# Tomeu7/AO-MARL

Measured on AMD Instinct MI355X. Metric: env steps/sec (AO frames/sec), higher is better.
Workload: dtype f32

## Files before the change

### ao_marl_amd/csrc/aomarl_capi.hip

```cpp
#include "aomarl_kernels.hip"

#include <math.h>
#include <stdlib.h>
#include <stdarg.h>
#include <stdio.h>
#include <string.h>

#include <algorithm>
#include <climits>
#include <string>
#include <vector>

static thread_local char g_err[512] = "";

int fail(const char *fmt, ...) {
  va_list ap;
  va_start(ap, fmt);
  vsnprintf(g_err, sizeof(g_err), fmt, ap);
  va_end(ap);
  return 1;
}


struct aomarl_ctx {
  DevSys sys;
  std::vector<void *> owned;
  int nlayers = 0, ndm = 0;
  int dim[AOMARL_MAX_LAYERS], ns[AOMARL_MAX_LAYERS], abclass[AOMARL_MAX_LAYERS];
  float deltax[AOMARL_MAX_LAYERS], deltay[AOMARL_MAX_LAYERS];
  int nclass = 0;
  int maxdim = 0, maxK = 0;
  float gain = 0.f, delay = 0.f;
  bool spot_fast = false;
  bool force_generic_dm = false, force_valu_target = false;
  bool force_generic_spot = false, force_generic_target = false, force_unfused_frame = false;
  int dft_mode = -1;
  bool reset_untransposed = false;
  int small_chain = 1;
  hipEvent_t ride_ev = nullptr;
  bool rode = false;
  int residual_shortcut = 0;
  bool skip_do_control = false;
  int small_move = 1;
  bool small_ok = false;
  int reset_streams = 2;
  bool reset_prefetch_whole = true;
  hipEvent_t ev_reset = nullptr, ev_reset2[3] = {nullptr, nullptr, nullptr};
  bool no_extrude_sg = false;
  bool defer_dm_shape = false;
  int fused_debug = 0;
  bool prefetch_atmos = false, premoved = false;
  bool frame_wait_pending = false;
  bool screens_dirty_main = true;
  float cmat_scale = 1.f, v2m_scale = 1.f, m2v_scale = 1.f, s2m_scale = 1.f, ab_scale[AOMARL_MAX_LAYERS] = {1.f, 1.f, 1.f, 1.f, 1.f, 1.f, 1.f, 1.f};
  bool subpixel_flow = false;
  float frac_x[AOMARL_MAX_LAYERS] = {0, 0, 0, 0, 0, 0, 0, 0}, frac_y[AOMARL_MAX_LAYERS] = {0, 0, 0, 0, 0, 0, 0, 0};
  bool graph_step = false, capturing = false, side_joined = false, fork_recorded = false;
  hipEvent_t ev_fork = nullptr;
  struct StepGraph { std::vector<long long> key; hipGraphExec_t exec; hipGraph_t graph; unsigned long long arith[AR_N]; int fw_variant[6]; };
  std::vector<StepGraph> graphs;
  unsigned long long graph_hits = 0, graph_captures = 0;
  unsigned long long cfg_epoch = 0;
  const int32_t *sel_checked = nullptr;
  int sel_checked_n = 0, sel_checked_nm = 0;
  int fw_variant[6] = {0, 0, 0, 0, 0, 0};
  char fw_name[96] = {0};
  bool time_fw = false;
  std::vector<hipEvent_t> fw_ev;
  size_t fw_ev_used = 0;
  std::vector<hipEvent_t> fw_ev_retired;
  hipStream_t atm_stream = nullptr, psf_stream = nullptr;
  hipEvent_t ev_frame = nullptr, ev_moved = nullptr, ev_psf = nullptr;
  hipEvent_t ev_frame_cur = nullptr;
  bool frame_marked = false;
  struct FramePipe {
    bool have_twin = false, active = false;
    const float *owner_screens = nullptr;
    aomarl_state twin;
    int par = 0;
    hipStream_t fstream = nullptr;
    hipEvent_t ev_cmd = nullptr, ev_commit = nullptr, ev_done[2] = {nullptr, nullptr}, ev_psf[2] = {nullptr, nullptr};
    hipEvent_t ev_done_cur[2] = {nullptr, nullptr};
    bool psf_out[2] = {false, false};
// ... 396 lines not shown
      std::vector<int32_t> tinfo(tsub.size(), 0);
      for (int r = 0; r < nt; r++)
        for (int t = 0; t < nt; t++) {
          const int32_t sb = tsub[(size_t)r * nt + t];
          bool full = true;
          for (int yy = 0; yy < 16; yy++) full = full && tmask[(size_t)(16 * r + yy) * nt + t] == 0xFFFF;
          int32_t v = 0;
          if (sb != -2) v |= 0x10000;
          if (full) v |= 0x20000;
          if (sb >= 0) { v |= 0x40000 | sb; v |= 0x10000; }
          tinfo[(size_t)r * nt + t] = v;
        }
      UP(int32_t, tinfo.data(), tinfo.size(), s.tile_info);
      {
        if (nt > 127) { aomarl_destroy(c); return fail("pupil too wide for the frame kernel's tile list"); }
        std::vector<int32_t> linfo((size_t)nt * (nt + 8), 0), lcount(nt, 0);
        for (int r = 0; r < nt; r++) {
          int k = 0;
          for (int t = 0; t < nt; t++)
            if (tinfo[(size_t)r * nt + t] & 0x10000) linfo[(size_t)r * (nt + 8) + k++] = tinfo[(size_t)r * nt + t] | (t << 24);
          lcount[r] = k;
          for (int kk = k; kk < nt + 8; kk++) linfo[(size_t)r * (nt + 8) + kk] = k ? linfo[(size_t)r * (nt + 8) + k - 1] : 0;
        }
        UP(int32_t, linfo.data(), linfo.size(), s.lit_info);
        UP(int32_t, lcount.data(), lcount.size(), s.lit_count);
        const int npm = (nt + 1) / 2 + 2;
        std::vector<int32_t> pinfo((size_t)nt * npm * 2, 0), pcount(nt, 0);
        for (int r = 0; r < nt; r++) {
          int k = 0;
          int32_t *row = &pinfo[(size_t)r * npm * 2];
          for (int g = 0; 2 * g < nt; g++) {
            const int ta = 2 * g, tb = 2 * g + 1 < nt ? 2 * g + 1 : 2 * g;
            const int32_t va = tinfo[(size_t)r * nt + ta], vb = 2 * g + 1 < nt ? tinfo[(size_t)r * nt + tb] : 0;
            if (!((va | vb) & 0x10000)) continue;
            row[2 * k] = ((va & 0x10000) ? va : 0) | (ta << 24);
            row[2 * k + 1] = ((vb & 0x10000) ? vb : 0) | (tb << 24);
            k++;
          }
          pcount[r] = k;
          for (int kk = k; kk < npm; kk++) {
            row[2 * kk] = k ? row[2 * (k - 1)] : 0;
            row[2 * kk + 1] = k ? row[2 * (k - 1) + 1] : 0;
          }
        }
        UP(int32_t, pinfo.data(), pinfo.size(), s.pair_info);
        UP(int32_t, pcount.data(), pcount.size(), s.pair_count);
      }
      {
        std::vector<int32_t> order(nt), work(nt, 0);
        for (int r = 0; r < nt; r++) {
          order[r] = r;
          for (int t = 0; t < nt; t++) {
            const int32_t v = tinfo[(size_t)r * nt + t];
            work[r] += (v & 0x10000) ? ((v & 0x40000) ? 4 : 1) : 0;
          }
        }
        std::stable_sort(order.begin(), order.end(), [&](int a, int b) { return work[a] > work[b]; });
        UP(int32_t, order.data(), order.size(), s.stripe_order);
      }
      {
        std::vector<_Float16> tw((size_t)nt * 64 * 8);
        std::vector<float> twf((size_t)nt * 64 * 4);
        for (int t = 0; t < nt; t++)
          for (int lane = 0; lane < 64; lane++)
            for (int j = 0; j < 4; j++) {
              const int x = 16 * t + 4 * (lane >> 4) + j, cc = lane & 15;
              const int k = cc < 8 ? cc + 1 : cc - 7;
              const double th = 2.0 * M_PI * (double)(((long long)k * x) % d->npsf) / (double)d->npsf;
              const float v = (float)(cc < 8 ? cos(th) : sin(th));
              const _Float16 hi = (_Float16)v;
              const _Float16 lo = (_Float16)(v - (float)hi);
              _Float16 *o = &tw[((size_t)t * 64 + lane) * 8];
              o[j] = hi; o[4 + j] = lo;
              twf[((size_t)t * 64 + lane) * 4 + j] = v;
            }
        const _Float16 *dev = nullptr;
        UP(_Float16, tw.data(), tw.size(), dev);
        s.psf_tw_h = dev;
        const float *devf = nullptr;
        UP(float, twf.data(), twf.size(), devf);
        s.psf_tw_f = devf;
      }
      {
        std::vector<float> z(64 * 8, 0.f);
        float *qt;
        UP(float, z.data(), z.size(), qt);
        hipLaunchKernelGGL(k_fill_qf_tab, dim3(1), dim3(128), 0, 0, qt);
        if (hipGetLastError() != hipSuccess || hipDeviceSynchronize() != hipSuccess) { aomarl_destroy(c); return fail("create: quadratic-form constants"); }
        s.qf_tab = qt;
      }
      UP(uint16_t, tmask.data(), tmask.size(), s.tile_mask);
      {
        const DevDm &T = s.dms[1];
        std::vector<float> tp((size_t)pd * pd * 2);
        for (int y = 0; y < pd; y++)
          for (int g = 0; g < pd / 4; g++)
            for (int j = 0; j < 4; j++) {
              const size_t o = (size_t)(y + T.toy) * T.dim + T.tox + 4 * g + j;
              float *dst = &tp[((size_t)y * (pd / 4) + g) * 8];
              dst[j] = c->h_tt[2 * o]; dst[4 + j] = c->h_tt[2 * o + 1];
            }
        UP(float, tp.data(), tp.size(), s.tt_pk);
      }
      s.fused_ok = 1; s.ntiles = nt;
      const DevDm &Z = s.dms[0];
      s.otf_ok = 0;
      if (Z.sep && Z.pitch > 0 && 16 % Z.pitch == 0) {
        auto first = [&](int p0, int pmin) {
          const int num = p0 - pmin - (Z.ss - 1);
          return num >= 0 ? (num + Z.pitch - 1) / Z.pitch : -((-num) / Z.pitch);
        };
        s.otf_gx0 = first(Z.tox, Z.i1min); s.otf_gy0 = first(Z.toy, Z.j1min);
        s.otf_xoff = Z.tox - (Z.i1min + Z.pitch * s.otf_gx0);
        s.otf_yoff = Z.toy - (Z.j1min + Z.pitch * s.otf_gy0);
        const int cnt = std::max((s.otf_xoff + 15) / Z.pitch + 1, (s.otf_yoff + 15) / Z.pitch + 1);
        s.otf_nb = (cnt + 3) / 4; s.otf_tpn = 16 / Z.pitch;
        s.otf_latw = (nt - 1) * s.otf_tpn + 4 * s.otf_nb;
        s.otf_ok = (s.otf_nb >= 1 && s.otf_nb <= 2 && s.otf_xoff >= 0 && s.otf_yoff >= 0) ? 1 : 0;
      }
    }
  }
#undef UP
  *out = c;
  return 0;
}

int aomarl_destroy(aomarl_ctx *c) {
  if (c)
    for (auto &sg : c->graphs) { (void)hipGraphExecDestroy(sg.exec); (void)hipGraphDestroy(sg.graph); }
  if (c) c->graphs.clear();
  if (!c) return 0;
  for (void *p : c->owned) (void)hipFree(p);
  for (int k = 0; k < 2; k++) {
    if (c->pipe.snap[k]) (void)hipFree(c->pipe.snap[k]);
    if (c->pipe.ev_done[k]) (void)hipEventDestroy(c->pipe.ev_done[k]);
    if (c->pipe.ev_psf[k]) (void)hipEventDestroy(c->pipe.ev_psf[k]);
  }
  if (c->ev_reset) (void)hipEventDestroy(c->ev_reset);
  for (int k = 0; k < 3; k++) if (c->ev_reset2[k]) (void)hipEventDestroy(c->ev_reset2[k]);
  if (c->pipe.ev_cmd) (void)hipEventDestroy(c->pipe.ev_cmd);
  if (c->pipe.ev_commit) (void)hipEventDestroy(c->pipe.ev_commit);
  if (c->pipe.fstream) { (void)hipStreamSynchronize(c->pipe.fstream); (void)hipStreamDestroy(c->pipe.fstream); }
  if (c->atm_stream) (void)hipStreamSynchronize(c->atm_stream);
  if (c->psf_stream) (void)hipStreamSynchronize(c->psf_stream);
  if (c->ev_frame) (void)hipEventDestroy(c->ev_frame);
  if (c->ev_moved) (void)hipEventDestroy(c->ev_moved);
  if (c->ev_psf) (void)hipEventDestroy(c->ev_psf);
  if (c->env_gain) (void)hipFree(c->env_gain);
  if (c->seed_stage) (void)hipFree(c->seed_stage);
  rp_free(c);
  if (c->timg) (void)hipFree(c->timg);
  for (hipEvent_t e : c->fw_ev) (void)hipEventDestroy(e);
  for (hipEvent_t e : c->fw_ev_retired) (void)hipEventDestroy(e);
  delete c;
  return 0;
}

static int replace_dev(aomarl_ctx *c, float **slot, const std::vector<float> &h) {
  if (*slot) {
    for (size_t i = 0; i < c->owned.size(); i++)
      if (c->owned[i] == *slot) { c->owned.erase(c->owned.begin() + i); break; }
    (void)hipFree(*slot);
    *slot = nullptr;
  }
  return upload<float>(c, h.data(), h.size(), slot);
}

int aomarl_set_cmat(aomarl_ctx *c, const float *cmat) {
  if (c) c->cfg_epoch++;
  if (!c || !cmat) return fail("aomarl_set_cmat: null argument");
  const int na = c->sys.nactu, nsl = c->sys.nslope;
// ... 176 lines not shown
```

### ao_marl_amd/csrc/aomarl_kernels.hip

```cpp
#include "aomarl_host.h"
#include "aomarl_gemm_p.h"
#include <type_traits>

#define WAVE 64

typedef unsigned u32x4 __attribute__((ext_vector_type(4)));

__device__ __forceinline__ hx2 cvt_h2(float a, float b) {
  return __builtin_bit_cast(hx2, __builtin_amdgcn_cvt_pkrtz(a, b));
}
__device__ __forceinline__ float sub_lo(hx2 h, float a) {
  float r;
  asm("v_fma_mix_f32 %0, %1, -1.0, %2 op_sel_hi:[1,0,0]" : "=v"(r) : "v"(h), "v"(a));
  return r;
}
__device__ __forceinline__ float sub_hi(hx2 h, float a) {
  float r;
  asm("v_fma_mix_f32 %0, %1, -1.0, %2 op_sel:[1,0,0] op_sel_hi:[1,0,0]" : "=v"(r) : "v"(h), "v"(a));
  return r;
}

struct __attribute__((packed, aligned(4))) f4u { float v[4]; };
__device__ __forceinline__ void add4(float acc[4], const float *p) {
  const f4u t = *reinterpret_cast<const f4u *>(p);
// ... 1368 lines not shown
  f32x2 d;
  asm volatile("v_pk_fma_f32 %0, %1, %2, %3" : "=v"(d) : "v"(a), "s"(bs), "v"(c));
  return d;
}
__device__ __forceinline__ f32x2 pk_fma_nc_s(f32x2 a, f32x2 bs, f32x2 c) {
  f32x2 d;
  asm volatile("v_pk_fma_f32 %0, %1, %2, %3 neg_lo:[0,0,1] neg_hi:[0,0,1]" : "=v"(d) : "v"(a), "s"(bs), "v"(c));
  return d;
}
__device__ __forceinline__ f32x2 pk_mul_s(f32x2 a, f32x2 bs) {
  f32x2 d;
  asm volatile("v_pk_mul_f32 %0, %1, %2" : "=v"(d) : "v"(a), "s"(bs));
  return d;
}

__device__ __forceinline__ void spot_cog_f32_pk(const DevSys &sys, const DevState &st, int e, int i, int lane,
                                                const float (&Cc)[4], const float (&Ss)[4], const float (&br)[4],
                                                const float (&bi)[4], int do_cog, const f32x4 z4) {
  const int q = lane >> 4, c = lane & 15;
  f32x4 PCr = z4, PCi = z4, PSr = z4, PSi = z4;
#pragma unroll
  for (int s = 0; s < 4; s++) {
    PCr = mfma16(br[s], Cc[s], PCr);
    PCi = mfma16(bi[s], Cc[s], PCi);
    PSr = mfma16(br[s], Ss[s], PSr);
    PSi = mfma16(bi[s], Ss[s], PSi);
  }
  PK_GUARD_MFMA();
  const f32x2 tr0l = pk_add(pk_lo(PCr), pk_lo(PSi)), ti0l = pk_sub(pk_lo(PCi), pk_lo(PSr));
  const f32x2 tr0h = pk_add(pk_hi(PCr), pk_hi(PSi)), ti0h = pk_sub(pk_hi(PCi), pk_hi(PSr));
  const f32x2 tr1l = pk_sub(pk_lo(PCr), pk_lo(PSi)), ti1l = pk_add(pk_lo(PCi), pk_lo(PSr));
  const f32x2 tr1h = pk_sub(pk_hi(PCr), pk_hi(PSi)), ti1h = pk_add(pk_hi(PCi), pk_hi(PSr));
  PK_END_TO_MFMA();
  const f32x4 TrA[2] = {pk_join(tr0l, tr0h), pk_join(tr1l, tr1h)};
  const f32x4 TiA[2] = {pk_join(ti0l, ti0h), pk_join(ti1l, ti1h)};
  f32x2 Pa[2], Pb[2];
  f32x2 Da, Db;
#pragma unroll
  for (int m = 0; m < 2; m++) {
    const f32x4 Tr = TrA[m], Ti = TiA[m];
    f32x4 QCr = z4, QCi = z4, QSr = z4, QSi = z4;
#pragma unroll
    for (int s = 0; s < 4; s++) {
      QCr = mfma16(Cc[s], Tr[s], QCr);
      QCi = mfma16(Cc[s], Ti[s], QCi);
      QSr = mfma16(Ss[s], Tr[s], QSr);
      QSi = mfma16(Ss[s], Ti[s], QSi);
    }
    PK_GUARD_MFMA();
    const f32x2 crl = pk_lo(QCr), crh = pk_hi(QCr), cil = pk_lo(QCi), cih = pk_hi(QCi);
    const f32x2 srl = pk_lo(QSr), srh = pk_hi(QSr), sil = pk_lo(QSi), sih = pk_hi(QSi);
    f32x2 pa = pk_mul(crl, crl), pb = pk_mul(crh, crh);
    if (m == 0) { Da = pk_mul(crl, sil); Db = pk_mul(crh, sih); }
    else { pk_acc_fma(Da, crl, sil); pk_acc_fma(Db, crh, sih); }
    pk_acc_fma(pa, sil, sil); pk_acc_fma(pb, sih, sih);
    pk_acc_fnma(Da, cil, srl); pk_acc_fnma(Db, cih, srh);
    pk_acc_fma(pa, cil, cil); pk_acc_fma(pb, cih, cih);
    pk_acc_fma(pa, srl, srl); pk_acc_fma(pb, srh, srh);
    Pa[m] = pa; Pb[m] = pb;
    __builtin_amdgcn_sched_barrier(0);
  }
  const f32x2 P0 = pk_add(Pa[0], Pb[0]), P1 = pk_add(Pa[1], Pb[1]);
  const float Xp = (float)(8 + (c >> 1)), Xm = (float)(7 - (c >> 1));
  const float p0 = P0.x + P0.y, p1 = P1.x + P1.y, da = Da.x + Da.y, db = Db.x + Db.y;
  float s0 = p0 + p1;
  float sx = fmaf(Xm, p1, Xp * p0);
  float sy = fmaf((float)(3 + 4 * q), db, fmaf((float)(1 + 4 * q), da, 7.5f * s0));
  s0 = wave_sum_last(s0);
  sx = wave_sum_last(sx);
  sy = wave_sum_last(sy);
  if (do_cog && lane == 63) {
    float *sl = st.slopes + (long long)e * sys.nslope;
    if (s0 > 0.f) {
      const float inv = __builtin_amdgcn_rcpf(s0);
      sl[i] = (sx * inv - sys.cog_offset) * sys.cog_scale;
      sl[sys.nvalid + i] = (sy * inv - sys.cog_offset) * sys.cog_scale;
    } else {
      sl[i] = 0.f;
      sl[sys.nvalid + i] = 0.f;
    }
  }
}

struct SpotQf { f32x2 Ml, Mh, Sl, Sh; };

__device__ __forceinline__ SpotQf spot_qf_consts(int lane, const float2 *sTw ) {
  const int q = lane >> 4, c = lane & 15;
  float m[4], sv[4];
#pragma unroll
  for (int s = 0; s < 4; s++) {
    const int d = c - (4 * q + s);
    float a = 0.f, b = 0.f;
    for (int j = 0; j < 16; j++) {
      const float2 w = sTw[((2 * j + 1) * d) & 127];
      a += w.x;
      b = fmaf(0.5f + (float)(j >> 1), w.y, b);
    }
    m[s] = (d != 0 && (d & 1) == 0) ? 0.f : 2.f * a;
    sv[s] = 2.f * b;
  }
  SpotQf k;
  k.Ml = f32x2{m[0], m[1]}; k.Mh = f32x2{m[2], m[3]};
  k.Sl = f32x2{sv[0], sv[1]}; k.Sh = f32x2{sv[2], sv[3]};
  return k;
}

__global__ __launch_bounds__(128) void k_fill_qf_tab(float *__restrict__ tab) {
  __shared__ float2 sTw[128];
  const int tid = threadIdx.x;
  float sn, cs;
  sincospif((float)tid * (1.0f / 64.0f), &sn, &cs);
  sTw[tid] = make_float2(cs, sn);
  __syncthreads();
  if (tid < 64) {
    const SpotQf k = spot_qf_consts(tid, sTw);
    float *o = tab + 8 * tid;
    o[0] = k.Ml.x; o[1] = k.Ml.y; o[2] = k.Mh.x; o[3] = k.Mh.y;
    o[4] = k.Sl.x; o[5] = k.Sl.y; o[6] = k.Sh.x; o[7] = k.Sh.y;
  }
}

typedef unsigned u32x2 __attribute__((ext_vector_type(2)));
#ifndef FW_QF6_PK
#define FW_QF6_PK 1
#endif
#ifndef FW_QF6_ACC2
#define FW_QF6_ACC2 0
#endif
__device__ __forceinline__ float swap32_add(float a, float b) {
  const u32x2 t = __builtin_amdgcn_permlane32_swap(__float_as_uint(a), __float_as_uint(b), false, false);
  return __uint_as_float(t[0]) + __uint_as_float(t[1]);
}
__device__ __forceinline__ float swap16_add(float a, float b) {
  const u32x2 t = __builtin_amdgcn_permlane16_swap(__float_as_uint(a), __float_as_uint(b), false, false);
  return __uint_as_float(t[0]) + __uint_as_float(t[1]);
}
__device__ __forceinline__ float spot_qf_moments(const SpotQf &K, const float (&er)[4], const float (&ei)[4], const f32x4 z4) {
  const float Mc[4] = {K.Ml.x, K.Ml.y, K.Mh.x, K.Mh.y}, Sc[4] = {K.Sl.x, K.Sl.y, K.Sh.x, K.Sh.y};
  f32x4 Wr = z4, Wi = z4, V = z4;
#pragma unroll
  for (int s = 0; s < 4; s++) {
    Wr = mfma16(Mc[s], er[s], Wr);
    Wi = mfma16(Mc[s], ei[s], Wi);
    V = mfma16(Sc[s], er[s], V);
  }
#if FW_QF6_PK
  const f32x2 er01 = {er[0], er[1]}, er23 = {er[2], er[3]}, ei01 = {ei[0], ei[1]}, ei23 = {ei[2], ei[3]};
  __builtin_amdgcn_sched_barrier(0);
  const f32x2 a01 = pk_add(er01, ei01), a23 = pk_add(er23, ei23);
  const f32x2 b01 = pk_sub(ei01, er01), b23 = pk_sub(ei23, er23);
  PK_END_TO_MFMA();
  const float A[4] = {a01.x, a01.y, a23.x, a23.y}, B[4] = {b01.x, b01.y, b23.x, b23.y};
#else
  float A[4], B[4];
#pragma unroll
  for (int s = 0; s < 4; s++) { A[s] = er[s] + ei[s]; B[s] = ei[s] - er[s]; }
#endif
#if FW_QF6_ACC2
  f32x4 Xa = z4, Xb = z4, G3 = z4;
#pragma unroll
  for (int s = 0; s < 4; s++) {
    Xa = mfma16(A[s], Wr[s], Xa);
    Xb = mfma16(B[s], Wi[s], Xb);
    G3 = mfma16(ei[s], V[s], G3);
  }
  PK_GUARD_MFMA();
  const f32x2 Xl = pk_add(pk_lo(Xa), pk_lo(Xb)), Xh = pk_add(pk_hi(Xa), pk_hi(Xb));
#else
  f32x4 X = z4, G3 = z4;
#pragma unroll
  for (int s = 0; s < 4; s++) {
    X = mfma16(A[s], Wr[s], X);
    G3 = mfma16(ei[s], V[s], G3);
    X = mfma16(B[s], Wi[s], X);
  }
  PK_GUARD_MFMA();
  const f32x2 Xl = pk_lo(X), Xh = pk_hi(X);
#endif
  f32x2 p0 = pk_mul(Xl, K.Ml);
  f32x2 px = pk_mul(pk_lo(G3), K.Ml);
  f32x2 py = pk_mul(Xl, K.Sl);
  pk_acc_fma(p0, Xh, K.Mh);
  pk_acc_fma(px, pk_hi(G3), K.Mh);
  pk_acc_fma(py, Xh, K.Sh);
  const float s0 = p0.x + p0.y, tx = px.x + px.y, ty = py.x + py.y;
  float z = swap16_add(swap32_add(s0, tx), swap32_add(ty, p0.y));
  z += dpp_f<0xB1>(z);
  z += dpp_f<0x4E>(z);
  z += dpp_f<0x141>(z);
  z += dpp_f<0x140>(z);
  return z;
}
__device__ __forceinline__ void qf_slopes(const DevSys &sys, float s0, float tx, float ty, float &sx, float &sy) {
  if (s0 > 0.f) {
    const float inv = __builtin_amdgcn_rcpf(s0);
    sx = (fmaf(tx, 2.f * inv, 7.5f) - sys.cog_offset) * sys.cog_scale;
    sy = (fmaf(-ty, inv, 7.5f) - sys.cog_offset) * sys.cog_scale;
  } else {
    sx = 0.f; sy = 0.f;
  }
}

template <bool NOISE, bool WRITE_CUBE>
__device__ __forceinline__ void spot_finish_v(const DevSys &sys, const DevState &st, int e, int i,
                                              int lane, const float (&v)[2][2][2], int do_cog,
                                              float flux_i) {
  const int q = lane >> 4, c = lane & 15;
  const bool owner = (c & 1) == 0;
  float tot = 0.f;
#pragma unroll
  for (int sy = 0; sy < 2; sy++)
#pragma unroll
    for (int sx = 0; sx < 2; sx++)
#pragma unroll
      for (int h = 0; h < 2; h++) tot += v[sy][sx][h];
  const int Xp = 8 + (c >> 1), Xm = 7 - (c >> 1);
  if (!NOISE && !WRITE_CUBE) {
    const float A0 = (v[0][0][0] + v[0][0][1]) + (v[1][0][0] + v[1][0][1]);
    const float A1 = (v[0][1][0] + v[0][1][1]) + (v[1][1][0] + v[1][1][1]);
    float sx_ = (float)Xp * A0;
    sx_ = fmaf((float)Xm, A1, sx_);
    float sy_ = (float)(8 + 2 * q) * (v[0][0][0] + v[0][1][0]);
    sy_ = fmaf((float)(9 + 2 * q), v[0][0][1] + v[0][1][1], sy_);
    sy_ = fmaf((float)(7 - 2 * q), v[1][0][0] + v[1][1][0], sy_);
    sy_ = fmaf((float)(6 - 2 * q), v[1][0][1] + v[1][1][1], sy_);
    tot = wave_sum_last(A0 + A1);
    sx_ = wave_sum_last(sx_);
    sy_ = wave_sum_last(sy_);
    if (do_cog && lane == 63) {
      float *sl = st.slopes + (long long)e * sys.nslope;
      if (tot > 0.f) {
        const float inv = __builtin_amdgcn_rcpf(tot);
        sl[i] = (sx_ * inv - sys.cog_offset) * sys.cog_scale;
        sl[sys.nvalid + i] = (sy_ * inv - sys.cog_offset) * sys.cog_scale;
      } else {
        sl[i] = 0.f;
        sl[sys.nvalid + i] = 0.f;
      }
    }
    (void)flux_i;
    return;
  }
  tot = wave_sum(owner ? tot : 0.f);
  const float g = tot > 0.f ? sys.nphot * flux_i / tot : 0.f;
  float s0 = 0.f, sx = 0.f, sy = 0.f;
  if (NOISE) {
    const int hh = c & 1;
    const uint32_t sd = st.seeds[e], fr = st.frame[e];
#pragma unroll
    for (int ty_ = 0; ty_ < 2; ty_++)
#pragma unroll
      for (int tx_ = 0; tx_ < 2; tx_++) {
        const int Y = ty_ ? 7 - (2 * q + hh) : 8 + 2 * q + hh, X = tx_ ? Xm : Xp;
        const uint32_t idx = (uint32_t)i * 256u + (uint32_t)(Y * 16 + X);
        const float val = sh_noise((hh ? v[ty_][tx_][1] : v[ty_][tx_][0]) * g, sys.noise, sd, fr, idx);
        if (WRITE_CUBE) st.bincube[((long long)e * sys.nvalid + i) * 256 + Y * 16 + X] = val;
        s0 += val;
        sx += val * (float)X;
        sy += val * (float)Y;
      }
  } else {
#pragma unroll
    for (int ty_ = 0; ty_ < 2; ty_++)
#pragma unroll
      for (int tx_ = 0; tx_ < 2; tx_++)
#pragma unroll
        for (int h = 0; h < 2; h++) {
          const int Y = ty_ ? 7 - (2 * q + h) : 8 + 2 * q + h, X = tx_ ? Xm : Xp;
// ... 417 lines not shown
#define FW_FULL 0x20000
#define FW_SUB 0x40000
__device__ __forceinline__ float sci_rev(float ph, float inv_lambda) { return ph * inv_lambda; }

typedef const int __attribute__((address_space(4))) *const_int_p;
typedef const float __attribute__((address_space(4))) *const_float_p;

template <int NL, bool OTF>
struct FrameRaw {
  float L[NL][4];
  float P[OTF ? 1 : 4], T[8];
  unsigned mrow;
  float F;
  f4u SH;
  float4 CS;
};

template <int NL, int NB, bool OTF, bool NOISE, bool WRITE_CUBE, bool HP>
#ifndef FW_WAVES
#define FW_WAVES 3
#endif
#ifndef FW_QF
#define FW_QF 1
#endif
#ifndef FW_DMA
#define FW_DMA 1
#endif
#ifndef FW_DEPTH
#define FW_DEPTH 2
#endif
#ifndef FW_DMA_F32
#define FW_DMA_F32 1
#endif
#ifndef FW_SLOTS1
#define FW_SLOTS1 0
#endif
#define FW_SLOT_BYTES(dma) ((dma) ? (FW_SLOTS1 ? 2 * 3 * 1024 : 16384) : 16384)
#define FWD_BLK 1152
#define FWD_IMG (2 * 1024 + 128)
#define FWD_WAVE(nl) ((nl) * FWD_IMG)
__global__ __launch_bounds__(256) __attribute__((amdgpu_waves_per_eu(FW_WAVES, FW_WAVES)))
void k_frame_wave(DevSys sys, DevState st, int env_begin,
                                                    int env_count, int do_cog,
                                                    float *__restrict__ TR,
                                                    float *__restrict__ TPART, int nblk) {
  extern __shared__ float smem[];
  const int pd = sys.pupdiam, ntl = sys.ntiles;
  const int tid = threadIdx.x, lane = tid & 63, q = lane >> 4, c = lane & 15;
  const int wv = __builtin_amdgcn_readfirstlane(tid >> 6);
  constexpr bool QF = FW_QF && OTF && !HP && !NOISE && !WRITE_CUBE;
  constexpr bool DMA = FW_DMA && OTF && (HP || FW_DMA_F32);
  float2 *sTw = reinterpret_cast<float2 *>(smem);
  float *lat_all = reinterpret_cast<float *>(sTw + (QF ? 0 : 128));
  float4 *shb = reinterpret_cast<float4 *>(lat_all + 4 * 4 * NB * (OTF ? sys.otf_latw : 0));
  char *dimg = reinterpret_cast<char *>(shb) + FW_SLOT_BYTES(DMA) + (DMA ? wv * FWD_WAVE(NL) : 0);
  float4 *qmom = reinterpret_cast<float4 *>(reinterpret_cast<char *>(shb) + FW_SLOT_BYTES(DMA) + (DMA ? 4 * FWD_WAVE(NL) : 0)) + wv * ntl;
  const int dbg = do_cog >> 8;
  do_cog &= 1;
  const int r = sys.stripe_order[blockIdx.y];
  const int el = 4 * blockIdx.x + wv;
  if constexpr (!QF) {
    if (tid < 128) {
      float sn, cs;
      sincospif((float)tid * (1.0f / 64.0f), &sn, &cs);
      sTw[tid] = make_float2(cs, sn);
    }
    __syncthreads();
  }
  const bool active = el < env_count;
  const int e = env_begin + (active ? el : env_count - 1);
  float Cc[4] = {0.f, 0.f, 0.f, 0.f}, Ss[4] = {0.f, 0.f, 0.f, 0.f};
  if constexpr (!QF) {
#pragma unroll
    for (int s = 0; s < 4; s++) {
      const float2 w = sTw[((4 * q + s) * (2 * c + 1)) & 127];
      Cc[s] = w.x; Ss[s] = w.y;
    }
  }
  SpotTwH twh;
  if (HP) twh = spot_tw_h(Cc, Ss);
  SpotQf qfk;
  if constexpr (QF) {
    const float4 ka = reinterpret_cast<const float4 *>(sys.qf_tab)[2 * lane], kb = reinterpret_cast<const float4 *>(sys.qf_tab)[2 * lane + 1];
    qfk.Ml = f32x2{ka.x, ka.y}; qfk.Mh = f32x2{ka.z, ka.w};
    qfk.Sl = f32x2{kb.x, kb.y}; qfk.Sh = f32x2{kb.z, kb.w};
  }
  unsigned shstep;
  const int y = 16 * r + c;
  const char *layb[NL];
  __amdgpu_buffer_rsrc_t lrs[NL];
  unsigned lpxs[NL], ldim[NL], lvo[NL];
#pragma unroll
  for (int l = 0; l < NL; l++) {
    const DevLayer &L = sys.layers[l];
    layb[l] = reinterpret_cast<const char *>(st.screens + (long long)e * sys.screen_stride + L.screen_off);
    lrs[l] = __builtin_amdgcn_make_buffer_rsrc(const_cast<char *>(layb[l]), 0,
                                               4 * L.dim * (L.dim + RING_PAD), 0x00020000);
    ldim[l] = (unsigned)L.dim;
    int px = L.tox + st.origin[(e * sys.nlayers + l) * 2]; px -= (px >= L.dim) ? L.dim : 0;
    int py = L.toy + st.origin[(e * sys.nlayers + l) * 2 + 1]; py -= (py >= L.dim) ? L.dim : 0;
    lpxs[l] = (unsigned)px;
    unsigned pr = (unsigned)y + (unsigned)py; pr = min(pr, pr - ldim[l]);
    lvo[l] = 4u * (pr * (ldim[l] + RING_PAD) + 4u * (unsigned)q);
  }
  const DevDm &D0 = sys.dms[0], &D1 = sys.dms[1];
  const float *pzt = st.dm_shape + (long long)e * sys.shape_stride + D0.shape_off;
  const float *ttslot = st.dm_shape + (long long)e * sys.shape_stride + D1.shape_off;
  const float c0 = ttslot[0], c1 = ttslot[1];
  const int half = pd / 2;
  const unsigned pvo = 4u * ((unsigned)(y + D0.toy) * (unsigned)D0.dim + (unsigned)D0.tox + 4u * (unsigned)q);
  const unsigned tvo = 32u * ((unsigned)y * (unsigned)(pd >> 2) + (unsigned)q);
  const unsigned mvo = 2u * (unsigned)y * (unsigned)ntl;
  const char *pztb = reinterpret_cast<const char *>(pzt);
  const char *ttb = reinterpret_cast<const char *>(sys.tt_pk);
  const char *mkb = reinterpret_cast<const char *>(sys.tile_mask);
  const bool sh_tt = wv < 2;
  const void *shbase = sh_tt ? static_cast<const void *>(ttb) : (HP ? sys.psf_tw_h : sys.psf_tw_f);
  const __amdgpu_buffer_rsrc_t shrs = __builtin_amdgcn_make_buffer_rsrc(
      const_cast<void *>(shbase), 0, sh_tt ? 8 * pd * pd : ntl * 1024, 0x00020000);
  const unsigned shvo = sh_tt ? tvo + 16u * (unsigned)wv : 16u * (unsigned)lane;
  shstep = sh_tt ? 7u : 10u;
  float pivot;
  {
    float v = OTF ? ttslot[2] : pzt[(half + D0.toy) * D0.dim + half + D0.tox];
    const float2 f = reinterpret_cast<const float2 *>(D1.influ)[(half + D1.toy) * D1.dim + half + D1.tox];
    v += c0 * f.x + c1 * f.y;
#pragma unroll
    for (int l = 0; l < NL; l++) {
      const DevLayer &L = sys.layers[l];
      int py = L.toy + st.origin[(e * sys.nlayers + l) * 2 + 1]; py -= (py >= L.dim) ? L.dim : 0;
      unsigned pyc = (unsigned)(half + py); pyc = min(pyc, pyc - ldim[l]);
      unsigned pxc = (unsigned)half + lpxs[l]; pxc = min(pxc, pxc - ldim[l]);
      v += reinterpret_cast<const float *>(layb[l])[pyc * (ldim[l] + RING_PAD) + pxc];
    }
    pivot = v;
  }
  float Pxr[NB], Pyr[NB];
  const int jm = (c >> 2) + 4 * (c & 3);
  const bool jm_ok = jm < 4 * NB;
  const int latw = sys.otf_latw, tpn = sys.otf_tpn;
  float *lat = lat_all + wv * (4 * NB * latw);
  if (OTF) {
#pragma unroll
    for (int s = 0; s < NB; s++) {
      const int ax = sys.otf_xoff + c - D0.pitch * (q + 4 * s);
      const int ay = sys.otf_yoff + c - D0.pitch * (q + 4 * s);
      Pxr[s] = (ax >= 0 && ax < D0.ss) ? D0.prof[ax] : 0.f;
      Pyr[s] = (ay >= 0 && ay < D0.ss) ? D0.prof[ay] : 0.f;
    }
    const float *volt = st.voltage + (long long)e * st.ld_actu + D0.com_off;
    for (int i = 0; i < 4 * NB; i++) {
      const int gy = sys.otf_gy0 + r * tpn + i;
      for (int jj = lane; jj < latw; jj += 64) {
        const int gx = sys.otf_gx0 + jj;
        float v = 0.f;
        if (gx >= 0 && gx < D0.gw && gy >= 0 && gy < D0.gh) {
          const int a = D0.grid[gy * D0.gw + gx];
          if (a >= 0) v = volt[a];
        }
        lat[i * latw + jj] = v;
      }
    }
    __builtin_amdgcn_wave_barrier();
  }
  const float *latq = lat + (jm_ok ? jm : 0);
  const float wfs_il = sys.wfs_inv_lambda, tar_il = sys.tar_inv_lambda;
  const f32x4 Z4 = opaque_zero4();
  f32x4 PA = {0.f, 0.f, 0.f, 0.f}, PB = {0.f, 0.f, 0.f, 0.f};
// ... 1146 lines not shown
```

Measured before the change: 549,900.

## Factor spot quadratic-form moments through a host-built orthogonal basis

Replaces the quadratic-form moment computation with a factorization: a symmetric basis H (from SVD and Jacobi eigen-decomposition on the host) projects the field, and the moments become sums of squares and cross terms of the projected vectors. The kernel goes from 20 MFMAs plus packed add/sub to 16 MFMAs and a few DPP multiply-accumulates, with constants built once on the host instead of by a setup kernel. It adds a fair amount of host numerical code and relies on the factorization reproducing the original moments to within float rounding.

Measured after the change: 570,500, median of 6. 1.04x the previous value.

```diff
diff --git a/ao_marl_amd/csrc/aomarl_capi.hip b/ao_marl_amd/csrc/aomarl_capi.hip
--- a/ao_marl_amd/csrc/aomarl_capi.hip
+++ b/ao_marl_amd/csrc/aomarl_capi.hip
@@ -1,4 +1,5 @@
 #include "aomarl_kernels.hip"
+#include "aomarl_qf4_host.h"
 
 #include <math.h>
 #include <stdlib.h>
@@ -561,11 +562,10 @@
         s.psf_tw_f = devf;
       }
       {
-        std::vector<float> z(64 * 8, 0.f);
-        float *qt;
-        UP(float, z.data(), z.size(), qt);
-        hipLaunchKernelGGL(k_fill_qf_tab, dim3(1), dim3(128), 0, 0, qt);
-        if (hipGetLastError() != hipSuccess || hipDeviceSynchronize() != hipSuccess) { aomarl_destroy(c); return fail("create: quadratic-form constants"); }
+        float qtab[64 * 8];
+        if (!aomarl_qf4::build_table(qtab)) { aomarl_destroy(c); return fail("create: quadratic-form constants"); }
+        const float *qt = nullptr;
+        UP(float, qtab, 64 * 8, qt);
         s.qf_tab = qt;
       }
       UP(uint16_t, tmask.data(), tmask.size(), s.tile_mask);
diff --git a/ao_marl_amd/csrc/aomarl_kernels.hip b/ao_marl_amd/csrc/aomarl_kernels.hip
--- a/ao_marl_amd/csrc/aomarl_kernels.hip
+++ b/ao_marl_amd/csrc/aomarl_kernels.hip
@@ -1474,51 +1474,9 @@
   }
 }
 
-struct SpotQf { f32x2 Ml, Mh, Sl, Sh; };
-
-__device__ __forceinline__ SpotQf spot_qf_consts(int lane, const float2 *sTw ) {
-  const int q = lane >> 4, c = lane & 15;
-  float m[4], sv[4];
-#pragma unroll
-  for (int s = 0; s < 4; s++) {
-    const int d = c - (4 * q + s);
-    float a = 0.f, b = 0.f;
-    for (int j = 0; j < 16; j++) {
-      const float2 w = sTw[((2 * j + 1) * d) & 127];
-      a += w.x;
-      b = fmaf(0.5f + (float)(j >> 1), w.y, b);
-    }
-    m[s] = (d != 0 && (d & 1) == 0) ? 0.f : 2.f * a;
-    sv[s] = 2.f * b;
-  }
-  SpotQf k;
-  k.Ml = f32x2{m[0], m[1]}; k.Mh = f32x2{m[2], m[3]};
-  k.Sl = f32x2{sv[0], sv[1]}; k.Sh = f32x2{sv[2], sv[3]};
-  return k;
-}
-
-__global__ __launch_bounds__(128) void k_fill_qf_tab(float *__restrict__ tab) {
-  __shared__ float2 sTw[128];
-  const int tid = threadIdx.x;
-  float sn, cs;
-  sincospif((float)tid * (1.0f / 64.0f), &sn, &cs);
-  sTw[tid] = make_float2(cs, sn);
-  __syncthreads();
-  if (tid < 64) {
-    const SpotQf k = spot_qf_consts(tid, sTw);
-    float *o = tab + 8 * tid;
-    o[0] = k.Ml.x; o[1] = k.Ml.y; o[2] = k.Mh.x; o[3] = k.Mh.y;
-    o[4] = k.Sl.x; o[5] = k.Sl.y; o[6] = k.Sh.x; o[7] = k.Sh.y;
-  }
-}
+struct SpotQf { f32x4 h; f32x2 ky; float kx; };
 
 typedef unsigned u32x2 __attribute__((ext_vector_type(2)));
-#ifndef FW_QF6_PK
-#define FW_QF6_PK 1
-#endif
-#ifndef FW_QF6_ACC2
-#define FW_QF6_ACC2 0
-#endif
 __device__ __forceinline__ float swap32_add(float a, float b) {
   const u32x2 t = __builtin_amdgcn_permlane32_swap(__float_as_uint(a), __float_as_uint(b), false, false);
   return __uint_as_float(t[0]) + __uint_as_float(t[1]);
@@ -1527,55 +1485,42 @@
   const u32x2 t = __builtin_amdgcn_permlane16_swap(__float_as_uint(a), __float_as_uint(b), false, false);
   return __uint_as_float(t[0]) + __uint_as_float(t[1]);
 }
+__device__ __forceinline__ float dpp4e_mul(float a, float b) {
+  float d;
+  asm volatile("v_mul_f32_dpp %0, %1, %2 quad_perm:[2,3,0,1] row_mask:0xf bank_mask:0xf bound_ctrl:1" : "=v"(d) : "v"(a), "v"(b));
+  return d;
+}
+__device__ __forceinline__ void dpp4e_fmac(float &acc, float a, float b) {
+  asm volatile("v_fmac_f32_dpp %0, %1, %2 quad_perm:[2,3,0,1] row_mask:0xf bank_mask:0xf bound_ctrl:1" : "+v"(acc) : "v"(a), "v"(b));
+}
 __device__ __forceinline__ float spot_qf_moments(const SpotQf &K, const float (&er)[4], const float (&ei)[4], const f32x4 z4) {
-  const float Mc[4] = {K.Ml.x, K.Ml.y, K.Mh.x, K.Mh.y}, Sc[4] = {K.Sl.x, K.Sl.y, K.Sh.x, K.Sh.y};
-  f32x4 Wr = z4, Wi = z4, V = z4;
+  f32x4 Dr = z4, Di = z4;
 #pragma unroll
   for (int s = 0; s < 4; s++) {
-    Wr = mfma16(Mc[s], er[s], Wr);
-    Wi = mfma16(Mc[s], ei[s], Wi);
-    V = mfma16(Sc[s], er[s], V);
-  }
-#if FW_QF6_PK
-  const f32x2 er01 = {er[0], er[1]}, er23 = {er[2], er[3]}, ei01 = {ei[0], ei[1]}, ei23 = {ei[2], ei[3]};
+    Dr = mfma16(er[s], K.h[s], Dr);
+    Di = mfma16(ei[s], K.h[s], Di);
+  }
+  f32x4 Pr = z4, Pi = z4;
+#pragma unroll
+  for (int r = 0; r < 4; r++) {
+    Pr = mfma16(K.h[r], Dr[r], Pr);
+    Pi = mfma16(K.h[r], Di[r], Pi);
+  }
+  PK_GUARD_MFMA();
+  const f32x2 rl = pk_lo(Pr), rh = pk_hi(Pr), il = pk_lo(Pi), ih = pk_hi(Pi);
+  f32x2 p0 = pk_mul(rl, rl);
+  f32x2 py = pk_mul(il, rh);
+  float px = dpp4e_mul(Pr[0], Pi[0]);
+  pk_acc_fma(p0, rh, rh);
+  pk_acc_fnma(py, ih, rl);
+  dpp4e_fmac(px, Pr[1], Pi[1]);
+  pk_acc_fma(p0, il, il);
+  py = pk_mul(py, K.ky);
+  dpp4e_fmac(px, Pr[2], Pi[2]);
+  pk_acc_fma(p0, ih, ih);
+  dpp4e_fmac(px, Pr[3], Pi[3]);
   __builtin_amdgcn_sched_barrier(0);
-  const f32x2 a01 = pk_add(er01, ei01), a23 = pk_add(er23, ei23);
-  const f32x2 b01 = pk_sub(ei01, er01), b23 = pk_sub(ei23, er23);
-  PK_END_TO_MFMA();
-  const float A[4] = {a01.x, a01.y, a23.x, a23.y}, B[4] = {b01.x, b01.y, b23.x, b23.y};
-#else
-  float A[4], B[4];
-#pragma unroll
-  for (int s = 0; s < 4; s++) { A[s] = er[s] + ei[s]; B[s] = ei[s] - er[s]; }
-#endif
-#if FW_QF6_ACC2
-  f32x4 Xa = z4, Xb = z4, G3 = z4;
-#pragma unroll
-  for (int s = 0; s < 4; s++) {
-    Xa = mfma16(A[s], Wr[s], Xa);
-    Xb = mfma16(B[s], Wi[s], Xb);
-    G3 = mfma16(ei[s], V[s], G3);
-  }
-  PK_GUARD_MFMA();
-  const f32x2 Xl = pk_add(pk_lo(Xa), pk_lo(Xb)), Xh = pk_add(pk_hi(Xa), pk_hi(Xb));
-#else
-  f32x4 X = z4, G3 = z4;
-#pragma unroll
-  for (int s = 0; s < 4; s++) {
-    X = mfma16(A[s], Wr[s], X);
-    G3 = mfma16(ei[s], V[s], G3);
-    X = mfma16(B[s], Wi[s], X);
-  }
-  PK_GUARD_MFMA();
-  const f32x2 Xl = pk_lo(X), Xh = pk_hi(X);
-#endif
-  f32x2 p0 = pk_mul(Xl, K.Ml);
-  f32x2 px = pk_mul(pk_lo(G3), K.Ml);
-  f32x2 py = pk_mul(Xl, K.Sl);
-  pk_acc_fma(p0, Xh, K.Mh);
-  pk_acc_fma(px, pk_hi(G3), K.Mh);
-  pk_acc_fma(py, Xh, K.Sh);
-  const float s0 = p0.x + p0.y, tx = px.x + px.y, ty = py.x + py.y;
+  const float s0 = p0.x + p0.y, tx = px * K.kx, ty = py.x + py.y;
   float z = swap16_add(swap32_add(s0, tx), swap32_add(ty, p0.y));
   z += dpp_f<0xB1>(z);
   z += dpp_f<0x4E>(z);
@@ -2159,8 +2104,8 @@
   SpotQf qfk;
   if constexpr (QF) {
     const float4 ka = reinterpret_cast<const float4 *>(sys.qf_tab)[2 * lane], kb = reinterpret_cast<const float4 *>(sys.qf_tab)[2 * lane + 1];
-    qfk.Ml = f32x2{ka.x, ka.y}; qfk.Mh = f32x2{ka.z, ka.w};
-    qfk.Sl = f32x2{kb.x, kb.y}; qfk.Sh = f32x2{kb.z, kb.w};
+    qfk.h = f32x4{ka.x, ka.y, ka.z, ka.w};
+    qfk.ky = f32x2{kb.x, kb.y}; qfk.kx = kb.z;
   }
   unsigned shstep;
   const int y = 16 * r + c;
diff --git a/ao_marl_amd/csrc/aomarl_qf4_host.h b/ao_marl_amd/csrc/aomarl_qf4_host.h
--- /dev/null
+++ b/ao_marl_amd/csrc/aomarl_qf4_host.h
@@ -0,0 +1,197 @@
+#pragma once
+#include <cmath>
+#include <cstring>
+
+namespace aomarl_qf4 {
+
+constexpr int NX = 16;
+constexpr int NF = 16;
+constexpr int NR = 2 * NF;
+
+struct Basis {
+  double H[NX][NX];
+  double t[NX / 2];
+  double err_m, err_s;
+};
+
+inline void jacobi_sym(double (&A)[NX][NX], double (&W)[NX][NX]) {
+  for (int i = 0; i < NX; i++)
+    for (int j = 0; j < NX; j++) W[i][j] = i == j ? 1.0 : 0.0;
+  for (int sweep = 0; sweep < 100; sweep++) {
+    bool rotated = false;
+    for (int p = 0; p < NX - 1; p++)
+      for (int q = p + 1; q < NX; q++) {
+        const double apq = A[p][q];
+        if (std::fabs(apq) <= 1e-17 * std::sqrt(std::fabs(A[p][p] * A[q][q])) || apq == 0.0) continue;
+        rotated = true;
+        const double zeta = (A[q][q] - A[p][p]) / (2.0 * apq);
+        const double tn = (zeta >= 0.0 ? 1.0 : -1.0) / (std::fabs(zeta) + std::sqrt(1.0 + zeta * zeta));
+        const double cs = 1.0 / std::sqrt(1.0 + tn * tn), sn = cs * tn;
+        for (int k = 0; k < NX; k++) {
+          const double a = A[k][p], b = A[k][q];
+          A[k][p] = cs * a - sn * b; A[k][q] = sn * a + cs * b;
+        }
+        for (int k = 0; k < NX; k++) {
+          const double a = A[p][k], b = A[q][k];
+          A[p][k] = cs * a - sn * b; A[q][k] = sn * a + cs * b;
+        }
+        for (int k = 0; k < NX; k++) {
+          const double a = W[k][p], b = W[k][q];
+          W[k][p] = cs * a - sn * b; W[k][q] = sn * a + cs * b;
+        }
+      }
+    if (!rotated) break;
+  }
+}
+
+inline bool build_basis(Basis &out) {
+  const double PI = 3.14159265358979323846;
+  double A[NR][NX], U[NR][NR];
+  double V[NX][NX], u[NF];
+  std::memset(U, 0, sizeof U);
+  for (int j = 0; j < NF; j++) {
+    const double th = 2.0 * PI * (j + 0.5) / 64.0;
+    u[j] = 0.5 + (double)(j >> 1);
+    for (int x = 0; x < NX; x++) { A[2 * j][x] = std::cos(th * x); A[2 * j + 1][x] = std::sin(th * x); }
+    U[2 * j + 1][2 * j] = u[j]; U[2 * j][2 * j + 1] = -u[j];
+  }
+  for (int i = 0; i < NX; i++)
+    for (int j = 0; j < NX; j++) V[i][j] = i == j ? 1.0 : 0.0;
+  for (int sweep = 0; sweep < 100; sweep++) {
+    bool rotated = false;
+    for (int p = 0; p < NX - 1; p++)
+      for (int q = p + 1; q < NX; q++) {
+        double al = 0.0, be = 0.0, ga = 0.0;
+        for (int k = 0; k < NR; k++) { al += A[k][p] * A[k][p]; be += A[k][q] * A[k][q]; ga += A[k][p] * A[k][q]; }
+        if (std::fabs(ga) <= 1e-17 * std::sqrt(al * be)) continue;
+        rotated = true;
+        const double zeta = (be - al) / (2.0 * ga);
+        const double tn = (zeta >= 0.0 ? 1.0 : -1.0) / (std::fabs(zeta) + std::sqrt(1.0 + zeta * zeta));
+        const double cs = 1.0 / std::sqrt(1.0 + tn * tn), sn = cs * tn;
+        for (int k = 0; k < NR; k++) {
+          const double a = A[k][p], b = A[k][q];
+          A[k][p] = cs * a - sn * b; A[k][q] = sn * a + cs * b;
+        }
+        for (int k = 0; k < NX; k++) {
+          const double a = V[k][p], b = V[k][q];
+          V[k][p] = cs * a - sn * b; V[k][q] = sn * a + cs * b;
+        }
+      }
+    if (!rotated) break;
+  }
+  double H[NX][NX], sig[NX];
+  for (int i = 0; i < NX; i++) {
+    double n2 = 0.0;
+    for (int k = 0; k < NR; k++) n2 += A[k][i] * A[k][i];
+    sig[i] = std::sqrt(n2);
+    if (!(sig[i] > 0.0)) return false;
+    for (int k = 0; k < NR; k++) A[k][i] /= sig[i];
+    for (int x = 0; x < NX; x++) H[x][i] = std::sqrt(2.0) * V[x][i] * sig[i];
+  }
+  double T[NX][NX], B[NX][NX], W[NX][NX];
+  {
+    double UR[NR][NX];
+    for (int a = 0; a < NR; a++)
+      for (int i = 0; i < NX; i++) {
+        double s = 0.0;
+        for (int b = 0; b < NR; b++) s += U[a][b] * A[b][i];
+        UR[a][i] = s;
+      }
+    double G[NX][NX];
+    for (int i = 0; i < NX; i++)
+      for (int j = 0; j < NX; j++) {
+        double s = 0.0;
+        for (int a = 0; a < NR; a++) s += A[a][i] * UR[a][j];
+        G[i][j] = s;
+      }
+    for (int i = 0; i < NX; i++)
+      for (int j = 0; j < NX; j++) T[i][j] = 0.5 * (G[i][j] - G[j][i]);
+  }
+  for (int i = 0; i < NX; i++)
+    for (int j = 0; j < NX; j++) {
+      double s = 0.0;
+      for (int k = 0; k < NX; k++) s += T[k][i] * T[k][j];
+      B[i][j] = s;
+    }
+  for (int i = 0; i < NX; i++)
+    for (int j = i + 1; j < NX; j++) B[i][j] = B[j][i] = 0.5 * (B[i][j] + B[j][i]);
+  jacobi_sym(B, W);
+  int idx[NX];
+  for (int i = 0; i < NX; i++) idx[i] = i;
+  for (int i = 1; i < NX; i++)
+    for (int j = i; j > 0 && B[idx[j]][idx[j]] > B[idx[j - 1]][idx[j - 1]]; j--) { const int s = idx[j]; idx[j] = idx[j - 1]; idx[j - 1] = s; }
+  double Q[NX][NX];
+  auto clean = [&](double (&v)[NX], int ncol) {
+    for (int pass = 0; pass < 2; pass++)
+      for (int a = 0; a < ncol; a++) {
+        double d = 0.0;
+        for (int i = 0; i < NX; i++) d += v[i] * Q[i][a];
+        for (int i = 0; i < NX; i++) v[i] -= d * Q[i][a];
+      }
+    double n2 = 0.0;
+    for (int i = 0; i < NX; i++) n2 += v[i] * v[i];
+    return std::sqrt(n2);
+  };
+  for (int k = 0; k < NX / 2; k++) {
+    double w[NX], v[NX];
+    for (int i = 0; i < NX; i++) w[i] = W[i][idx[2 * k]];
+    double n = clean(w, 2 * k);
+    if (!(n > 0.5)) return false;
+    int big = 0;
+    for (int i = 1; i < NX; i++) if (std::fabs(w[i]) > std::fabs(w[big])) big = i;
+    if (w[big] < 0.0) n = -n;
+    for (int i = 0; i < NX; i++) { w[i] /= n; Q[i][2 * k + 1] = w[i]; }
+    for (int i = 0; i < NX; i++) {
+      double s = 0.0;
+      for (int j = 0; j < NX; j++) s += T[i][j] * w[j];
+      v[i] = s;
+    }
+    for (int i = 0; i < NX; i++) Q[i][2 * k] = 0.0;
+    const double tk = clean(v, 2 * k + 2);
+    if (!(tk > 0.0)) return false;
+    for (int i = 0; i < NX; i++) Q[i][2 * k] = v[i] / tk;
+    out.t[k] = tk;
+  }
+  for (int x = 0; x < NX; x++)
+    for (int a = 0; a < NX; a++) {
+      double s = 0.0;
+      for (int i = 0; i < NX; i++) s += H[x][i] * Q[i][a];
+      out.H[x][a] = s;
+    }
+  double em = 0.0, es = 0.0, nm = 0.0, ns = 0.0;
+  for (int xp = 0; xp < NX; xp++)
+    for (int x = 0; x < NX; x++) {
+      double m = 0.0, s = 0.0, hm = 0.0, hs = 0.0;
+      for (int j = 0; j < NF; j++) {
+        const double th = 2.0 * PI * (j + 0.5) / 64.0 * (double)(xp - x);
+        m += 2.0 * std::cos(th); s += 2.0 * u[j] * std::sin(th);
+      }
+      for (int a = 0; a < NX; a++) hm += out.H[xp][a] * out.H[x][a];
+      for (int k = 0; k < NX / 2; k++)
+        hs += out.t[k] * (out.H[xp][2 * k] * out.H[x][2 * k + 1] - out.H[xp][2 * k + 1] * out.H[x][2 * k]);
+      em += (hm - m) * (hm - m); nm += m * m;
+      es += (hs - s) * (hs - s); ns += s * s;
+    }
+  out.err_m = std::sqrt(em / nm); out.err_s = std::sqrt(es / ns);
+  return out.err_m <= 1e-12 && out.err_s <= 1e-12;
+}
+
+inline int lane_column(int c) { return (c & ~3) | ((c & 1) << 1) | ((c >> 1) & 1); }
+
+inline bool build_table(float (&tab)[64 * 8], Basis *basis = nullptr) {
+  Basis b;
+  const bool ok = build_basis(b);
+  if (basis) *basis = b;
+  if (!ok) return false;
+  for (int lane = 0; lane < 64; lane++) {
+    const int q = lane >> 4, a = lane_column(lane & 15);
+    float *o = tab + 8 * lane;
+    for (int s = 0; s < 4; s++) o[s] = (float)b.H[4 * q + s][a];
+    o[4] = (float)(-2.0 * b.t[2 * q]); o[5] = (float)(-2.0 * b.t[2 * q + 1]);
+    o[6] = (float)((a & 1) ? -b.t[a >> 1] : b.t[a >> 1]);
+    o[7] = 0.f;
+  }
+  return true;
+}
+
+}
```
